# fateshelled/sycl_points

Measured on AMD Instinct MI355X. Metric: gicp_correspondences_per_sec, higher is better.
Workload: dtype f32

## Files before the change

### sycl_points_amd/csrc/registration.hip

```cpp
#include <algorithm>
#include <mutex>

#include "registration_device.h"
#include "sp_cov_normal.h"

namespace sp {
namespace {


struct PointTerm {
    float H[6][6];
    float b[6];
    float sq;
    float residual_norm;
    float genz_weight;
};

__device__ __forceinline__ void se3_jacobian(const Rigid& T, float px, float py, float pz, float J[3][6]) {
#pragma unroll
    for (int i = 0; i < 3; ++i) {
        const float r0 = T.R[i][0], r1 = T.R[i][1], r2 = T.R[i][2];
        J[i][0] = chain3(r0, 0.0f, r1, pz, r2, -py);
        J[i][1] = chain3(r0, -pz, r1, 0.0f, r2, px);
        J[i][2] = chain3(r0, py, r1, -px, r2, 0.0f);
// ... 333 lines not shown
    if ((threadIdx.x & (kWave - 1)) == 0) {
        atomicAdd(&counts[0], inl);
        atomicAdd(&counts[1], pl);
    }
}

__global__ void gn_update_kernel(sp_linearized* lin, float* T, float lambda, float crit_rot, float crit_trans,
                                 float* delta_out8) {
    __shared__ LdltScratch ldlt_ws;
    if (threadIdx.x == 0 && blockIdx.x == 0) gn_update_impl(lin, T, lambda, crit_rot, crit_trans, delta_out8, true, ldlt_ws);
}


template <bool P2D>
__global__ __launch_bounds__(kBlock) void prepare_cov_kernel(const float4* __restrict__ covs, unsigned n,
                                                             const float4* __restrict__ order_pts,
                                                             const unsigned* __restrict__ order_idx,
                                                             float4* __restrict__ out,
                                                             const float* __restrict__ rho2 = nullptr) {
    const unsigned i = blockIdx.x * kBlock + threadIdx.x;
    if (i >= n) return;
    const unsigned src = order_pts ? __float_as_uint(order_pts[i].w) : (order_idx ? order_idx[i] : i);
    const Mat3 C = load_cov(covs + 4 * (size_t)src);
    const Mat3 P = P2D ? inverse(C) : plane_regularize(C);
    out[2 * (size_t)i] = make_float4(P.m[0][0], (P.m[0][1] + P.m[1][0]) * 0.5f, (P.m[0][2] + P.m[2][0]) * 0.5f, P.m[1][1]);
    out[2 * (size_t)i + 1] = make_float4((P.m[1][2] + P.m[2][1]) * 0.5f, P.m[2][2], rho2 ? rho2[src] : 0.0f, 0.0f);
}

__global__ __launch_bounds__(kBlock) void inverse_order_kernel(const float4* __restrict__ gpts, unsigned n,
                                                               unsigned* __restrict__ inv) {
    const unsigned i = blockIdx.x * kBlock + threadIdx.x;
    if (i < n) inv[__float_as_uint(gpts[i].w)] = i;
}
__global__ __launch_bounds__(kBlock) void certificate_kernel(const float4* __restrict__ gpts, unsigned n,
                                                             const int32_t* __restrict__ idx3,
                                                             const float* __restrict__ d23,
                                                             const unsigned* __restrict__ inv,
                                                             float* __restrict__ rho2, float4* __restrict__ nb, float bound2) {
    const unsigned i = blockIdx.x * kBlock + threadIdx.x;
    if (i >= n) return;
    const unsigned o = __float_as_uint(gpts[i].w);
    constexpr float kShrink = 0.25f * (1.0f - 1e-3f);
    rho2[o] = fminf(d23[3 * (size_t)i + 1], bound2) * kShrink;
    const int u1 = idx3[3 * (size_t)i + 1];
    float4 r = make_float4(INFINITY, INFINITY, INFINITY, 0.0f);
    if (u1 >= 0) {
        const float4 p = gpts[inv[u1]];
        r.x = p.x; r.y = p.y; r.z = p.z;
    }
    r.w = fminf(d23[3 * (size_t)i + 2], bound2) * kShrink;
    nb[i] = r;
}

__global__ __launch_bounds__(kBlock) void query_cell_kernel(const float4* __restrict__ pts, unsigned n, GridDesc g,
                                                            Mat4Arg T_val, const float* __restrict__ T_dev,
                                                            unsigned* __restrict__ keys, unsigned* __restrict__ vals) {
    const unsigned i = blockIdx.x * kBlock + threadIdx.x;
    if (i >= n) return;
    const Rigid T = load_rigid_colmajor(T_dev ? T_dev : T_val.m);
    const float4 p = pts[i];
    float qx, qy, qz;
    transform_point(T, p.x, p.y, p.z, qx, qy, qz);
    unsigned key = (unsigned)g.nx * g.ny * g.nz;
    if (isfinite(qx) && isfinite(qy) && isfinite(qz)) {
        const int cx = cell_coord(qx, g.ox, g.inv_h, g.nx), cy = cell_coord(qy, g.oy, g.inv_h, g.ny),
                  cz = cell_coord(qz, g.oz, g.inv_h, g.nz);
        key = ((unsigned)cz * g.ny + cy) * g.nx + cx;
    }
    keys[i] = key;
    vals[i] = i;
}
__global__ __launch_bounds__(kBlock) void prepare_source_kernel(const float4* __restrict__ pts,
                                                                const float4* __restrict__ covs,
                                                                unsigned* __restrict__ order, bool identity, unsigned n,
                                                                float* __restrict__ tiles) {
    const unsigned i = blockIdx.x * kBlock + threadIdx.x;
    if (i >= n) return;
    const unsigned src = identity ? i : order[i];
    if (identity) order[i] = i;
    const float4 p = pts[src];
    float* const w = tiles + ((size_t)(i / kWave) * kSrcTileWords + (i % kWave));
    w[0] = p.x; w[kWave] = p.y; w[2 * kWave] = p.z;
    if (!covs) return;
    const Mat3 P = plane_regularize(load_cov(covs + 4 * (size_t)src));
// ... 208 lines not shown
                xrow[r][e] = ok ? __uint_as_float((unsigned)v) : 0.0f;
            }
            __syncthreads();
            if (s_late) return false;
            if (threadIdx.x < kFanRow) {
                float sum = 0.0f;
                for (int r = 0; r < A.x.world; ++r) sum += xrow[r][threadIdx.x];
                red[1][threadIdx.x] = sum;
            }
        } else {
            const float rv = threadIdx.x < kFanRow ? A.fan_row_in[threadIdx.x] : 0.0f;
            after_loads();
            if (threadIdx.x < kFanRow) red[1][threadIdx.x] = rv;
        }
        __syncthreads();
        if (threadIdx.x < kAcc - 1) red[0][threadIdx.x] = red[1][threadIdx.x];
        else if (threadIdx.x == kAcc - 1)
            red[0][kAcc - 1] = __uint_as_float((unsigned)red[1][kAcc] * 4096u + (unsigned)red[1][kAcc - 1]);
        else if (threadIdx.x == kAcc) red[0][kAcc] = red[1][kAcc + 1];
        __syncthreads();
        return true;
    }
}
__device__ __forceinline__ void align_store_late_state(const AlignArgs& A) {
    if (threadIdx.x < kStateWords) {
        unsigned w = A.has_prev ? reinterpret_cast<const unsigned*>(A.state_in)[threadIdx.x] : 0u;
        if (!A.has_prev && threadIdx.x < 16) w = __float_as_uint(A.T_init[threadIdx.x]);
        if (threadIdx.x == kStateFlagWord) w = 1u;
        if (threadIdx.x == kStateFlagWord + 3) w = 1u;
        reinterpret_cast<unsigned*>(A.state_out)[threadIdx.x] = w;
    }
}

template <bool SHARDED>
__device__ __forceinline__ bool align_prologue(const AlignArgs& A, float* sT, unsigned* sflag) {
    __shared__ float red[kFinalThreads / 32][kPartial];
    __shared__ sp_linearized slin;
    __shared__ float sdelta[8];
    __shared__ LdltScratch ldlt_ws;
    if (A.first) {
        state_store(state_load(false, nullptr, A.T_init), sT, sflag);
        if (!SHARDED && blockIdx.x == 0 && A.searched_log && threadIdx.x >= 64 && threadIdx.x < 64 + kSearchedLog)
            A.searched_log[threadIdx.x - 64] = 0u;
        __syncthreads();
        return true;
    }
    const unsigned sv = state_load(A.has_prev, A.state_in, A.T_init);
    const unsigned nrows = (SHARDED && A.mode == ALIGN_ROWS) ? (unsigned)kAlignMaxBlocks : gridDim.x;
    const bool arrived = align_totals<SHARDED>(A, A.prev_rows, nrows, red, [=] { state_store(sv, sT, sflag); }, sflag);
    if (!arrived) {
        if (blockIdx.x == 0) align_store_late_state(A);
        return false;
    }
    auto zero_row = [&] {
        if (SHARDED && A.mode == ALIGN_FANIN && blockIdx.x == 0 && threadIdx.x >= 64 && threadIdx.x < 64 + kFanRow)
            A.fan_row_out[threadIdx.x - 64] = 0.0f;
    };
    if (sflag[0]) {
        if (blockIdx.x == 0 && threadIdx.x < kStateWords)
            reinterpret_cast<unsigned*>(A.state_out)[threadIdx.x] = reinterpret_cast<const unsigned*>(A.state_in)[threadIdx.x];
        zero_row();
        return false;
    }
    if (threadIdx.x == 0)
        finish_iteration(red[0], sT, A.lambda, A.crit_rot, A.crit_trans, sflag[1], &slin, sdelta, &ldlt_ws, blockIdx.x == 0, A.state_out,
                         A.searched_log,
                         A.k, A.lin_out);
    __syncthreads();
    if (sdelta[6] > 0.5f) {
        zero_row();
        return false;
    }
    return true;
}

template <int LOSS, bool FAST_NN, bool P2D = false, bool SHARDED = false>
__global__ __launch_bounds__(kAlignBlock) void gicp_align_kernel(FusedParams P, AlignArgs A,
                                                                 float* __restrict__ partials) {
    __shared__ float sT[16];
    __shared__ unsigned sflag[2];
    if (!align_prologue<SHARDED>(A, sT, sflag)) return;
    const Rigid T = uniform_pose(sT);
    float acc[kAcc - 1];
    unsigned cnt = 0, searched = 0;
    const unsigned stride = gridDim.x * kAlignBlock;
#pragma unroll
    for (int e = 0; e < kAcc - 1; ++e) acc[e] = 0.0f;
    const unsigned tile = xcd_tile();
    for (unsigned i = tile * kAlignBlock + threadIdx.x; i < P.n; i += stride)
        fused_point<LOSS, FAST_NN, P2D, kSeedSearches, kNegCert>(P, T, i, acc, cnt, searched);
    if constexpr (!SHARDED) {
        block_reduce_store<kAcc - 1, kAlignBlock>(acc, cnt, partials + (size_t)blockIdx.x * kPartial, false, searched);
    } else if (A.mode == ALIGN_ROWS) {
        block_reduce_store<kAcc - 1, kAlignBlock>(acc, cnt, partials + (size_t)blockIdx.x * kPartial, true, searched);
    } else {
        block_reduce_store<kAcc - 1, kAlignBlock, true>(acc, cnt, partials + (size_t)blockIdx.x * kPartial, false, searched);
        align_tail(A, partials);
    }
}

struct PersistArgs {
    AlignWs ws;
    unsigned* tickets;
    const float* T_init;
    float lambda, crit_rot, crit_trans;
    sp_linearized* lin_out;
    float* T_out;
    float* delta_out8;
    uint32_t* iterations_out;
    int max_iterations;
    int k_begin;
    int cache_valid_later;
    unsigned long long budget;
};
template <int LOSS, bool FAST_NN, bool P2D = false>
__global__ __launch_bounds__(kAlignBlock) void gicp_align_persistent_kernel(FusedParams P, PersistArgs A) {
    __shared__ float sT[16];
    __shared__ float red[kFinalThreads / 32][kPartial];
    __shared__ sp_linearized slin;
    __shared__ float sdelta[8];
    __shared__ LdltScratch ldlt_ws;
    __shared__ unsigned s_flag;
    const unsigned stride = gridDim.x * kAlignBlock;
    const unsigned tile = xcd_tile();
    __shared__ unsigned s_prev[2];
    if (A.k_begin >= 2) {
        if (threadIdx.x < 18) {
            const unsigned v = reinterpret_cast<const unsigned*>(&A.ws.state[A.k_begin & 1])[threadIdx.x < 16 ? threadIdx.x : kStateFlagWord + threadIdx.x - 16];
            if (threadIdx.x < 16) sT[threadIdx.x] = __uint_as_float(v);
            else s_prev[threadIdx.x - 16] = v;
        }
    } else {
        if (threadIdx.x < 16) sT[threadIdx.x] = A.T_init[threadIdx.x];
        else if (threadIdx.x < 18) s_prev[threadIdx.x - 16] = 0u;
    }
    if (A.k_begin == 0 && blockIdx.x == 0 && A.ws.searched_log && threadIdx.x >= 64 && threadIdx.x < 64 + kSearchedLog)
        A.ws.searched_log[threadIdx.x - 64] = 0u;
    __syncthreads();
    if (s_prev[0]) {
        if (blockIdx.x == 0) {
            const AlignState* const sp_ = &A.ws.state[A.k_begin & 1];
            if (threadIdx.x < kStateWords)
                reinterpret_cast<unsigned*>(&A.ws.state[(A.k_begin + 1) & 1])[threadIdx.x] = reinterpret_cast<const unsigned*>(sp_)[threadIdx.x];
            if (threadIdx.x < 16) A.T_out[threadIdx.x] = sp_->T[threadIdx.x];
            else if (threadIdx.x < 24 && A.delta_out8) A.delta_out8[threadIdx.x - 16] = sp_->delta[threadIdx.x - 16];
            else if (threadIdx.x == 24 && A.iterations_out) *A.iterations_out = sp_->iterations;
        }
        return;
    }
    unsigned iterations = s_prev[1];
    for (int k = A.k_begin;; ++k) {
        if (k > 0) {
            if (threadIdx.x == 0) s_flag = grid_wait(A.tickets, gridDim.x * (unsigned)(k - A.k_begin), A.budget) ? 0u : 2u;
            __syncthreads();
            if (s_flag == 2) {
                if (blockIdx.x == 0 && threadIdx.x < 16) A.T_out[threadIdx.x] = __int_as_float(0x7fc00000);
                if (blockIdx.x == 0 && threadIdx.x == 16 && A.iterations_out) *A.iterations_out = 0xffffffffu;
                if (blockIdx.x == 0 && threadIdx.x == 17) { A.ws.state[0].pad = 2u; A.ws.state[1].pad = 2u; }
                return;
            }
            reduce_rows_1024<true>(A.ws.part[(k - 1) & 1], gridDim.x, kAcc - 1, red, false, [] {});
            if (threadIdx.x == 0) {
                const bool publish = blockIdx.x == 0;
                AlignState* const so = &A.ws.state[(k - 1) & 1];
                if (publish) {
#pragma unroll
                    for (int i = 0; i < 16; ++i) so->T_lin[i] = sT[i];
                }
                unpack_totals(red[0], kAcc - 1, &slin);
                gn_update_impl(&slin, sT, A.lambda, A.crit_rot, A.crit_trans, sdelta, false, ldlt_ws);
                const bool conv = sdelta[6] > 0.5f;
                const bool last = conv || k == A.max_iterations;
                if (publish) {
                    const unsigned searched = (unsigned)red[0][kAcc];
#pragma unroll
                    for (int i = 0; i < 16; ++i) so->T[i] = sT[i];
#pragma unroll
                    for (int i = 0; i < 8; ++i) so->delta[i] = sdelta[i];
                    so->converged = conv ? 1u : 0u;
                    so->iterations = iterations + 1;
                    so->searched = searched;
                    so->pad = 0;
                    if (A.ws.searched_log && k - 1 < kSearchedLog) A.ws.searched_log[k - 1] = searched;
                    if (A.lin_out) *A.lin_out = slin;
                    if (last) {
                        A.ws.state[k & 1] = *so;
#pragma unroll
                        for (int i = 0; i < 16; ++i) A.T_out[i] = sT[i];
                        if (A.delta_out8)
#pragma unroll
                            for (int i = 0; i < 8; ++i) A.delta_out8[i] = sdelta[i];
                        if (A.iterations_out) *A.iterations_out = iterations + 1;
                    }
                }
                s_flag = last ? 1u : 0u;
            }
            __syncthreads();
            ++iterations;
            if (s_flag) return;
        }
        const Rigid T = uniform_pose(sT);
        float acc[kAcc - 1];
        unsigned cnt = 0, searched = 0;
#pragma unroll
        for (int e = 0; e < kAcc - 1; ++e) acc[e] = 0.0f;
        if (k == 1) P.cache_valid = A.cache_valid_later;
        for (unsigned i = tile * kAlignBlock + threadIdx.x; i < P.n; i += stride)
            fused_point<LOSS, FAST_NN, P2D, kSeedSearches, kNegCert>(P, T, i, acc, cnt, searched);
        block_reduce_store<kAcc - 1, kAlignBlock, true>(acc, cnt, A.ws.part[k & 1] + (size_t)blockIdx.x * kPartial, false, searched);
        grid_arrive(A.tickets);
        if (k == A.max_iterations - 1 && blockIdx.x != 0) return;
    }
}

struct AlignPublish {
    float* T_out;
    float* delta_out8;
    uint32_t* iterations_out;
    unsigned* xchg_epoch;
};
__device__ __forceinline__ void align_publish(const AlignState* state, const AlignPublish& Pb) {
    __threadfence();
    __syncthreads();
    if (!Pb.T_out) return;
    const unsigned* const w = reinterpret_cast<const unsigned*>(state);
    if (threadIdx.x < 16)
        reinterpret_cast<unsigned*>(Pb.T_out)[threadIdx.x] = __hip_atomic_load(w + threadIdx.x, __ATOMIC_RELAXED, __HIP_MEMORY_SCOPE_AGENT);
    else if (threadIdx.x < 24 && Pb.delta_out8)
        reinterpret_cast<unsigned*>(Pb.delta_out8)[threadIdx.x - 16] =
            __hip_atomic_load(w + 32 + (threadIdx.x - 16), __ATOMIC_RELAXED, __HIP_MEMORY_SCOPE_AGENT);
    else if (threadIdx.x == 24 && Pb.iterations_out)
        *Pb.iterations_out = __hip_atomic_load(w + kStateFlagWord + 1, __ATOMIC_RELAXED, __HIP_MEMORY_SCOPE_AGENT);
    else if (threadIdx.x == 32 && Pb.xchg_epoch)
        *Pb.xchg_epoch += 1u;
}
static_assert(offsetof(AlignState, delta) == 4 * 32, "AlignState layout");

__global__ __launch_bounds__(kFinalThreads) void align_solve_kernel(AlignArgs A, const float* __restrict__ rows,
                                                                    unsigned nrows, AlignPublish Pb) {
// ... 167 lines not shown
}
extern "C" int sp_genz_counts(const float* tgt_covs, const int32_t* nn_idx, const float* nn_d2, size_t n, float max_corr,
                              float planarity_threshold, uint32_t* counts_out, void* stream) {
    using namespace sp;
    hipStream_t st = as_stream(stream);
    if (zero_async(counts_out, 8, st) != SP_OK) return SP_ERR_HIP;
    if (n == 0) return SP_OK;
    genz_counts_kernel<<<reduce_grid(n), kBlock, 0, st>>>(reinterpret_cast<const float4*>(tgt_covs), nn_idx, nn_d2,
                                                          (unsigned)n, max_corr * max_corr, planarity_threshold,
                                                          counts_out);
    return launch_status();
}
extern "C" int sp_gn_update(sp_linearized* lin, float* T_dev, float lambda, float crit_rotation, float crit_translation,
                            float* delta_out8, void* stream) {
    sp::gn_update_kernel<<<1, 64, 0, sp::as_stream(stream)>>>(lin, T_dev, lambda, crit_rotation, crit_translation,
                                                              delta_out8);
    return sp::launch_status();
}
extern "C" int sp_gn_update_host(const sp_linearized* lin_host, float* T_host, float lambda, float crit_rotation,
                                 float crit_translation, float* delta_out8_host) {
    sp_linearized tmp = *lin_host;
    sp::LdltScratch w;
    sp::gn_update_impl(&tmp, T_host, lambda, crit_rotation, crit_translation, delta_out8_host, false, w);
    return SP_OK;
}



extern "C" void sp_gicp_target_destroy(sp_gicp_target* t) {
    if (!t) return;
    sp::pooled_free_after(t->covp, t->streams);
    sp::pooled_free_after(t->rho2, t->streams);
    sp::pooled_free_after(t->nb, t->streams);
    delete t;
}
extern "C" int sp_gicp_target_prepare(sp_gicp_target* t, const float* tgt_covs, int reg_type, void* stream) {
    using namespace sp;
    if (!t || !tgt_covs) {
        sp_set_error(reg_type == SP_REG_POINT_TO_DISTRIBUTION
                         ? "[Registration::validate_params] Covariance matrices of target must be pre-computed before "
                           "performing Point-to-Distribution ICP matching."
                         : "[Registration::validate_params] Covariance matrices of source and target must be pre-computed "
                           "before performing GICP matching.");
        return SP_ERR_RUNTIME;
    }
    if (reg_type != SP_REG_GICP && reg_type != SP_REG_POINT_TO_DISTRIBUTION) {
        sp_set_error("[sp_gicp_target_prepare] only RegType::GICP and RegType::POINT_TO_DISTRIBUTION have a prepared form");
        return SP_ERR_INVALID_ARGUMENT;
    }
    ++t->version;
    t->reg_type = reg_type;
    if (t->n == 0) return SP_OK;
    t->note(as_stream(stream));
    const float4* covs = reinterpret_cast<const float4*>(tgt_covs);
    if (reg_type == SP_REG_GICP)
        prepare_cov_kernel<false><<<div_up(t->n, kBlock), kBlock, 0, as_stream(stream)>>>(covs, (unsigned)t->n, t->grid->d_pts,
                                                                                          nullptr, t->covp, t->rho2);
    else
        prepare_cov_kernel<true><<<div_up(t->n, kBlock), kBlock, 0, as_stream(stream)>>>(covs, (unsigned)t->n, t->grid->d_pts,
                                                                                         nullptr, t->covp, t->rho2);
    return launch_status();
}
extern "C" int sp_gicp_target_update(sp_gicp_target* t, const float* tgt_covs, void* stream) {
    return sp_gicp_target_prepare(t, tgt_covs, t ? t->reg_type : SP_REG_GICP, stream);
}
namespace sp {
namespace {
int build_certificates(sp_gicp_target* t, hipStream_t st) {
    const sp_grid* const grid = t->grid;
    const size_t n = t->n;
    if (n == 0 || t->rho2 != nullptr) return SP_OK;
    ScratchBuf b_idx3, b_d23, b_inv;
    hipError_t e = pooled_alloc(&t->rho2, n * sizeof(float), st);
    if (e == hipSuccess) e = pooled_alloc(&t->nb, n * sizeof(float4), st);
    if (e == hipSuccess) e = b_idx3.get(n * 3 * sizeof(int32_t), st);
    if (e == hipSuccess) e = b_d23.get(n * 3 * sizeof(float), st);
    if (e == hipSuccess) e = b_inv.get(n * sizeof(unsigned), st);
    int32_t* const idx3 = b_idx3.as<int32_t>();
    float* const d23 = b_d23.as<float>();
    unsigned* const inv = b_inv.as<unsigned>();
    int rc = e == hipSuccess ? SP_OK : SP_ERR_HIP;
    const float bound2 = 9.0f * grid->h * grid->h;
    if (rc == SP_OK) rc = grid_search_own_points(grid, 3, idx3, d23, st, bound2);
    if (rc == SP_OK) {
        inverse_order_kernel<<<div_up(n, kBlock), kBlock, 0, st>>>(grid->d_pts, (unsigned)n, inv);
        certificate_kernel<<<div_up(n, kBlock), kBlock, 0, st>>>(grid->d_pts, (unsigned)n, idx3, d23, inv, t->rho2, t->nb, bound2);
        rc = launch_status();
    }
    if (hipStreamSynchronize(st) != hipSuccess && rc == SP_OK) rc = SP_ERR_HIP;
    if (rc != SP_OK) {
        if (e != hipSuccess) sp_set_error(hipGetErrorString(e));
        pooled_free(t->rho2); t->rho2 = nullptr;
        pooled_free(t->nb); t->nb = nullptr;
    }
    return rc;
}
int target_create(const sp_grid* grid, const float* tgt_covs, size_t n, bool certificates, void* stream, sp_gicp_target** out) {
    if (!out || !grid) return SP_ERR_INVALID_ARGUMENT;
    *out = nullptr;
    if (grid->n != n) {
        sp_set_error("[sp_gicp_target_create] the grid was built on a cloud of a different size");
        return SP_ERR_INVALID_ARGUMENT;
    }
    sp_gicp_target* t = new sp_gicp_target();
    t->grid = grid;
    t->n = n;
    t->note(as_stream(stream));
    if (n) {
        const hipError_t e = pooled_alloc(&t->covp, n * 2 * sizeof(float4), as_stream(stream));
        if (e != hipSuccess) {
            sp_set_error(hipGetErrorString(e));
            sp_gicp_target_destroy(t);
            return SP_ERR_HIP;
        }
    }
    if (certificates) {
        const int rc2 = build_certificates(t, as_stream(stream));
        if (rc2 != SP_OK) { sp_gicp_target_destroy(t); return rc2; }
    }
    const int rc = sp_gicp_target_update(t, tgt_covs, stream);
    if (rc != SP_OK) { sp_gicp_target_destroy(t); return rc; }
    *out = t;
    return SP_OK;
}
}
}
// ... 517 lines not shown
```

### sycl_points_amd/csrc/registration_device.h

```cpp
#ifndef SP_REGISTRATION_DEVICE_H
#define SP_REGISTRATION_DEVICE_H

#include "grid_device.h"
#include "radix_sort.h"
#include "sp_linearize.h"
#include "sp_xchg.h"

#include <type_traits>

void sp_set_error(const char* msg);

#include "sp_internal.h"

namespace sp {
namespace {

constexpr int kAcc = 29;
constexpr int kPartial = 32;
constexpr int kMaxBlocks = 1024;

template <bool SC1>
__device__ __forceinline__ void store_row_word(float* p, float v) {
    if (SC1) __hip_atomic_store(p, v, __ATOMIC_RELAXED, __HIP_MEMORY_SCOPE_AGENT);
    else *p = v;
}
template <bool SC1>
__device__ __forceinline__ float load_row_word(const float* p) {
    return SC1 ? __hip_atomic_load(p, __ATOMIC_RELAXED, __HIP_MEMORY_SCOPE_AGENT) : *p;
}
template <int NV, int BLOCK = kBlock, bool SC1 = false>
__device__ __forceinline__ void block_reduce_store(float (&acc)[NV], unsigned cnt, float* __restrict__ partial,
                                                   bool count_as_float = false, unsigned extra = 0) {
    __shared__ float red[BLOCK / kWave][kPartial];
    const unsigned lane = threadIdx.x & (kWave - 1), wave = threadIdx.x / kWave;
#pragma unroll
    for (int e = 0; e < NV; ++e) acc[e] = wave_sum_to_lane63(acc[e]);
    cnt = wave_sum_u32_to_lane63(cnt);
// ... 149 lines not shown
    for (int i = 0; i < 6; ++i) {
        H[i * 6 + i] = lin->H[i * 6 + i] + lambda * 1.0f;
        nb[i] = -lin->b[i];
    }
    const bool ok = ldlt6_solve(H, nb, delta, w);
    const float nr = sqrtf(delta[0] * delta[0] + delta[1] * delta[1] + delta[2] * delta[2]);
    const float nt = sqrtf(delta[3] * delta[3] + delta[4] * delta[4] + delta[5] * delta[5]);
    const bool conv = ok && (nr < crit_rot) && (nt < crit_trans);
    const Rigid cur = load_rigid_colmajor(T);
    const Rigid upd = rigid_mul(cur, se3_exp(delta));
    store_rigid_colmajor(upd, T);
    if (delta_out8) {
        for (int i = 0; i < 6; ++i) delta_out8[i] = delta[i];
        delta_out8[6] = conv ? 1.0f : 0.0f;
        delta_out8[7] = ok ? 1.0f : 0.0f;
    }
}

__device__ __forceinline__ Sym3 load_sym(const float4* __restrict__ p) {
    const float4 a = p[0], b = p[1];
    return Sym3{a.x, a.y, a.z, a.w, b.x, b.y};
}

constexpr unsigned kSrcPlanes = 9;
constexpr unsigned kSrcTileWords = kSrcPlanes * kWave;
__host__ __device__ inline size_t src_tile_words(size_t n) { return (n + kWave - 1) / kWave * kSrcTileWords; }

struct FusedParams {
    const float* src;
    const float4* tpts;
    const unsigned* tstart;
    const float4* tcovp;
    const float4* tnb;
    GridDesc g;
    unsigned n;
    float max_d2, scale;
    Mat4Arg T_val;
    const float* T_dev;
    const unsigned* perm;
    float4* ccache;
    int cache_valid;
    int32_t* nn_idx;
    float* nn_d2;
};

__device__ __forceinline__ const float* src_words(const FusedParams& P, unsigned i) {
    return P.src + ((size_t)(i / kWave) * kSrcTileWords + (i % kWave));
}
__device__ __forceinline__ float4 src_point(const float* __restrict__ w) {
    return make_float4(w[0], w[kWave], w[2 * kWave], 1.0f);
}
__device__ __forceinline__ Sym3 src_cov(const float* __restrict__ w) {
    return Sym3{w[3 * kWave], w[4 * kWave], w[5 * kWave], w[6 * kWave], w[7 * kWave], w[8 * kWave]};
}

template <int LOSS, bool P2D = false, bool ERR_ONLY = false, int NACC = kAcc - 1>
__device__ __forceinline__ void fused_math(const FusedParams& P, const Rigid& T, const float4 s, float qx, float qy,
                                           float qz, const Nearest& nn, const Sym3& Cs, const Sym3& Ct,
                                           float (&acc)[NACC], unsigned& cnt) {
    float t[NACC];
    linearize_terms<LOSS, P2D, ERR_ONLY>(T, s.x, s.y, s.z, qx, qy, qz, nn.x, nn.y, nn.z, Cs, Ct, P.scale, t);
#pragma unroll
    for (int e = 0; e < NACC; ++e) acc[e] += t[e];
    ++cnt;
}

// ... 5 lines not shown
    if (nn.idx >= 0) {
        const float4 c0 = P.tcovp[2 * (size_t)nn.pos], c1 = P.tcovp[2 * (size_t)nn.pos + 1];
        r0 = make_float4(nn.x, nn.y, nn.z, c1.z);
        r1 = c0;
        r2 = make_float4(c1.x, c1.y, __int_as_float(nn.idx), __uint_as_float(nn.pos));
        Ct = Sym3{c0.x, c0.y, c0.z, c0.w, c1.x, c1.y};
    }
    row[0] = r0;
    row[1] = r1;
    row[2] = r2;
}

__device__ __forceinline__ bool certified(const FusedParams& P, float d, float rho2, float qx, float qy, float qz,
                                          unsigned pos) {
    if (d < rho2) return true;
    if (!P.tnb || !(rho2 > 0.0f)) return false;
    const float4 nb = P.tnb[pos];
    return d < nb.w && d < dist2(qx, qy, qz, nb.x, nb.y, nb.z);
}

__device__ __forceinline__ float search_bound2(const FusedParams& P) {
    return (P.nn_idx == nullptr && P.max_d2 < FLT_MAX) ? __uint_as_float(__float_as_uint(P.max_d2) + 1u) : FLT_MAX;
}
__device__ __forceinline__ float search_bound2_margin(const FusedParams& P, float& margin2) {
    margin2 = 0.0f;
    if (P.nn_idx != nullptr || !(P.max_d2 < FLT_MAX) || P.ccache == nullptr) return search_bound2(P);
    const float B = sqrtf(P.max_d2), m = 0.25f * B;
    const float wide = (B + m) * (B + m);
    if (!(wide < FLT_MAX)) return search_bound2(P);
    margin2 = (0.98f * m) * (0.98f * m);
    return wide;
}

template <int LOSS, bool FAST_NN, bool P2D = false, bool SEED = true, bool NEG = true>
__device__ __forceinline__ void fused_point(const FusedParams& P, const Rigid& T, unsigned i, float (&acc)[kAcc - 1],
                                            unsigned& cnt, unsigned& searched) {
    const float* const sw = src_words(P, i);
    const float4 s = src_point(sw);
    float4* const row = P.ccache + 3 * (size_t)i;
    float qx, qy, qz;
    transform_point(T, s.x, s.y, s.z, qx, qy, qz);
    Nearest nn;
    Sym3 Ct{0.0f, 0.0f, 0.0f, 0.0f, 0.0f, 0.0f};
    bool hit = false;
    bool seeded = false;
    Nearest seed;
    seed.d2 = FLT_MAX; seed.idx = -1; seed.pos = 0; seed.x = seed.y = seed.z = 0.0f;
    if (P.cache_valid) {
        const float4 r0 = row[0], r1 = row[1], r2 = row[2];
        const float d = dist2(qx, qy, qz, r0.x, r0.y, r0.z);
        const unsigned pos = __float_as_uint(r2.w);
        if (certified(P, d, r0.w, qx, qy, qz, pos)) {
            hit = true;
            nn.idx = __float_as_int(r2.z); nn.pos = pos; nn.x = r0.x; nn.y = r0.y; nn.z = r0.z;
            nn.d2 = nn.idx >= 0 ? d : FLT_MAX;
            Ct = Sym3{r1.x, r1.y, r1.z, r1.w, r2.x, r2.y};
        } else if (SEED && __float_as_int(r2.z) >= 0) {
            seed.d2 = d; seed.idx = __float_as_int(r2.z); seed.pos = pos; seed.x = r0.x; seed.y = r0.y; seed.z = r0.z;
            seeded = true;
        }
    }
    if (!hit) {
        ++searched;
        float margin2 = 0.0f;
        const float bound2 = NEG ? search_bound2_margin(P, margin2) : search_bound2(P);
        seeded = seeded && seed.d2 < bound2;
        if (!seeded) { seed.d2 = bound2; seed.idx = -1; seed.pos = 0; seed.x = seed.y = seed.z = 0.0f; }
        if (FAST_NN) {
            nn = grid_nn1_auto(P.tpts, P.tstart, P.g, qx, qy, qz, bound2, &seed);
        } else {
            nn = grid_nn1(P.tpts, P.tstart, P.g, qx, qy, qz, &seed, 0);
        }
        if (NEG) store_correspondence(row, P, nn, Ct, qx, qy, qz, margin2);
        else store_correspondence(row, P, nn, Ct);
    }
    if (P.nn_idx) {
        const unsigned o = P.perm[i];
        P.nn_idx[o] = nn.idx;
        P.nn_d2[o] = nn.d2;
    }
    if (nn.idx < 0 || nn.d2 > P.max_d2) return;
    unsigned i_again = i;
    asm volatile("" : "+v"(i_again));
    const float* const sw_again = src_words(P, i_again);
    const Sym3 Cs = P2D ? Sym3{0.0f, 0.0f, 0.0f, 0.0f, 0.0f, 0.0f} : src_cov(sw_again);
    fused_math<LOSS, P2D>(P, T, src_point(sw_again), qx, qy, qz, nn, Cs, Ct, acc, cnt);
}

#ifdef SP_OPT_TIMING
__device__ unsigned long long g_sp_dbg[24 * 16];
__device__ unsigned g_sp_step;
__device__ unsigned long long g_sp_wg[24 * 8];
#define SP_PSTAMP(k) if (blockIdx.x == 0 && threadIdx.x == 0 && g_sp_step < 24) g_sp_dbg[g_sp_step * 16 + (k)] = wall_clock64()
#else
#define SP_PSTAMP(k)
#endif
template <int LOSS, bool P2D = false>
__device__ __forceinline__ void fused_point_wave(const FusedParams& P, const Rigid& T, unsigned i, bool valid,
                                                 float (&acc)[kAcc - 1], unsigned& cnt, unsigned& searched) {
    const unsigned ii = valid ? i : 0u;
    SP_PSTAMP(0);
    const float* const sw = src_words(P, ii);
    const float4 s = src_point(sw);
    float qx, qy, qz;
// ... 222 lines not shown
}

constexpr int kTicketShards = 8;
constexpr int kTicketStride = 32;
__device__ __forceinline__ void grid_arrive(unsigned* tickets) {
    if (threadIdx.x < kWave) {
        asm volatile("s_waitcnt vmcnt(0)" ::: "memory");
        if (threadIdx.x == 0)
            __hip_atomic_fetch_add(tickets + (blockIdx.x & (kTicketShards - 1)) * kTicketStride, 1u, __ATOMIC_RELAXED,
                                   __HIP_MEMORY_SCOPE_AGENT);
    }
}
__device__ __forceinline__ bool grid_wait(unsigned* tickets, unsigned want, unsigned long long budget) {
    const unsigned long long t0 = wall_clock64();
    for (;;) {
        unsigned have = 0;
#pragma unroll
        for (int sh = 0; sh < kTicketShards; ++sh)
            have += __hip_atomic_load(tickets + sh * kTicketStride, __ATOMIC_RELAXED, __HIP_MEMORY_SCOPE_AGENT);
        if (have >= want) return true;
        if (wall_clock64() - t0 > budget) return false;
        __builtin_amdgcn_s_sleep(2);
    }
}

}
}

struct sp_gicp_target {
    const sp_grid* grid = nullptr;
    float4* covp = nullptr;
    float* rho2 = nullptr;
    float4* nb = nullptr;
    unsigned long long version = 0;
    int reg_type = SP_REG_GICP;
    size_t n = 0;
    mutable sp::StreamSet streams;
    void note(hipStream_t st) const { streams.note(st); if (grid) sp::grid_use(grid, st); }
};
namespace sp {
constexpr size_t kOptRowsBytes = 2 * (size_t)256 * 32 * sizeof(unsigned long long);
}
struct sp_gicp_source {
    size_t n_max = 0, n = 0;
    float* tiles = nullptr;
    unsigned* perm = nullptr;
    float4* ccache = nullptr;
    float4* qcert = nullptr;
    float4* qcert2 = nullptr;
    size_t qcert_points = 0;
    mutable bool qcert_valid = false;
    float4* ccache2 = nullptr;
    unsigned long long* opt_rows = nullptr;
    mutable unsigned opt_epoch = 0;
    mutable bool cache_valid = false;
    const sp_gicp_target* cache_target = nullptr;
    unsigned long long cache_version = 0;
    bool sorted = false;
    int opt_stage_mask = 3;
    int opt_reuse = 2;
    int opt_fast_nn = -1;
    int opt_persistent = 1;
    int opt_persistent_from = 4;
    int opt_fuse_trials = 1;
    int opt_wave_query = 1;
    unsigned *keys_in = nullptr, *keys_out = nullptr, *vals_in = nullptr;
    void* sort_tmp = nullptr;
    size_t sort_tmp_bytes = 0;
};

namespace sp {
namespace {
FusedParams make_fused_params(const sp_gicp_target* target, const sp_gicp_source* source, const sp_factor_params* params,
                              const float* transT, int transT_on_device, int32_t* nn_idx_out, float* nn_d2_out) {
    const size_t n = source->n;
    FusedParams P;
    P.src = source->tiles;
    P.tpts = target->grid->d_pts;
    P.tstart = target->grid->d_start;
    P.tcovp = target->covp;
    P.tnb = source->opt_reuse > 1 ? target->nb : nullptr;
    P.g = grid_desc(target->grid);
    P.n = (unsigned)n;
    P.max_d2 = params->max_correspondence_distance * params->max_correspondence_distance;
    P.scale = params->robust_scale;
    for (int i = 0; i < 16; ++i) P.T_val.m[i] = (i % 5 == 0) ? 1.0f : 0.0f;
    if (transT && !transT_on_device)
        for (int i = 0; i < 16; ++i) P.T_val.m[i] = transT[i];
    P.T_dev = transT_on_device ? transT : nullptr;
    P.perm = source->perm;
    P.ccache = source->ccache;
    P.cache_valid = (source->opt_reuse && source->cache_valid && source->cache_target == target &&
                     source->cache_version == target->version) ? 1 : 0;
    P.nn_idx = (nn_idx_out && nn_d2_out) ? nn_idx_out : nullptr;
    P.nn_d2 = nn_d2_out;
    return P;
}

int check_prepared_reg(const sp_gicp_target* target, const sp_factor_params* params) {
    if (params->reg_type != SP_REG_GICP && params->reg_type != SP_REG_POINT_TO_DISTRIBUTION) {
        sp_set_error("[sp_gicp_*] only RegType::GICP and RegType::POINT_TO_DISTRIBUTION have a prepared/fused form");
        return SP_ERR_INVALID_ARGUMENT;
    }
    if (params->reg_type != target->reg_type) {
        sp_set_error("[sp_gicp_*] the prepared target holds the rows of another RegType: call sp_gicp_target_prepare");
        return SP_ERR_INVALID_ARGUMENT;
    }
    if (params->rotation_constraint_enable) {
        sp_set_error("[sp_gicp_*] the rotation constraint needs the raw covariances: use sp_gicp_linearize");
        return SP_ERR_INVALID_ARGUMENT;
    }
    return SP_OK;
}

// ... 79 lines not shown
```

### sycl_points_amd/csrc/registration_opt.hip

```cpp
#include <algorithm>

#include "sp_optimizer.h"

namespace sp {
namespace {

struct OptArgs {
    float* part[2];
    unsigned* tickets;
    unsigned long long* trows[2];
    unsigned tag_base;
    float4* rows[2];
    float4* qcert[2];
    int qcert_trusted;
    int fuse;
    const float* T_init;
    float* T_out;
    sp_opt_params opt;
    float scales[SP_OPT_MAX_LEVELS];
    int n_levels;
    int reuse;
    sp_align_result* result;
    unsigned long long budget;
};
// ... 162 lines not shown
#endif
    for (unsigned step = 0;; ++step) {
        const int phase = S.ctl.phase;
#ifdef SP_OPT_TIMING
        if (publish && threadIdx.x == 0) g_sp_step = step;
        __syncthreads();
#endif
        SP_STAMP(0);
        SP_WG_BEGIN();
        float* const row = A.part[step & 1] + (size_t)blockIdx.x * kPartial;
        [[maybe_unused]] float mine = 0.0f;
        if constexpr (WAVEQ) P.ccache = A.rows[S.ctl.cur];
        if (phase == PHASE_LIN) {
            P.scale = A.scales[S.ctl.level];
            P.cache_valid = S.ctl.cache_valid;
            const Rigid T = uniform_pose(S.sT);
            float acc[kAcc - 1];
            unsigned cnt = 0, searched = 0;
#pragma unroll
            for (int e = 0; e < kAcc - 1; ++e) acc[e] = 0.0f;
            if constexpr (WAVEQ) {
                const unsigned nw = BLOCK / kWave;
                const unsigned wave = (unsigned)__builtin_amdgcn_readfirstlane((int)(threadIdx.x / kWave));
                const bool qc_trust = A.qcert_trusted || S.ctl.n_lin > 0;
                for (unsigned i = blockIdx.x * nw + wave; i < P.n; i += gridDim.x * nw)
                    fused_query_wave<LOSS, P2D>(P, T, i, acc, cnt, searched, nullptr, qc_trust ? A.qcert[S.ctl.cur] : nullptr, A.qcert[S.ctl.cur]);
                SP_STAMP(4);
                mine = waveq_row_slot<kAcc - 1, BLOCK>(acc, cnt, searched, red);
            } else if constexpr (FAST_NN && BLOCK <= 256) {
                for (unsigned b = tile * BLOCK; b < P.n; b += stride)
                    fused_point_wave<LOSS, P2D>(P, T, b + threadIdx.x, b + threadIdx.x < P.n, acc, cnt, searched);
            } else {
                for (unsigned i = tile * BLOCK + threadIdx.x; i < P.n; i += stride)
                    fused_point<LOSS, FAST_NN, P2D, kSeedSearches, kNegCert>(P, T, i, acc, cnt, searched);
            }
            if constexpr (!WAVEQ) {
                SP_STAMP(4);
                if (single) block_reduce_lds<kAcc - 1, BLOCK>(acc, cnt, searched, red[0]);
                else block_reduce_store<kAcc - 1, BLOCK, true>(acc, cnt, row, false, searched);
            }
        } else if (WAVEQ && phase == PHASE_FUSED) {
            if constexpr (WAVEQ) {
                const Rigid T = uniform_pose(S.sTt);
                const Rigid TL = uniform_pose(S.sTlin);
                float acc[kAcc - 1], acc_t[1] = {0.0f};
                unsigned cnt = 0, searched = 0, cnt_t = 0;
#pragma unroll
                for (int e = 0; e < kAcc - 1; ++e) acc[e] = 0.0f;
                float4* const rows_out = A.rows[S.ctl.cur ^ 1];
                const float scale_trial = A.scales[S.ctl.level], scale_lin = A.scales[S.ctl.spec_level];
                const int reuse = S.reuse;
                const unsigned nw = BLOCK / kWave;
                const unsigned wave = (unsigned)__builtin_amdgcn_readfirstlane((int)(threadIdx.x / kWave));
                for (unsigned i = blockIdx.x * nw + wave; i < P.n; i += gridDim.x * nw) {
                    P.scale = scale_trial;
                    error_prepared_point<LOSS, P2D>(P, T, TL, i, acc_t, cnt_t);
                    P.scale = scale_lin;
                    P.cache_valid = reuse;
                    fused_query_wave<LOSS, P2D>(P, T, i, acc, cnt, searched, rows_out, A.qcert[S.ctl.cur], A.qcert[S.ctl.cur ^ 1]);
                }
                SP_STAMP(4);
                mine = waveq_row_slot<kAcc - 1, BLOCK>(acc, cnt, searched, red, acc_t[0], cnt_t);
            }
        } else {
            const Rigid T = uniform_pose(S.sTt);
            const Rigid TL = uniform_pose(S.sTlin);
            P.scale = A.scales[S.ctl.level];
// ... 207 lines not shown
```

Before: 32.09 billion.

## Add neighbor-list certificate to re-resolve cached correspondences without grid search

Target preparation now runs a self-kNN with more neighbors and records each target point's three nearest neighbors plus a certified radius. During alignment, a cached correspondence that fails the simple certificate can switch to a closer listed neighbor, or be kept, without a full grid NN search. The list path is enabled only when a per-iteration bound on pose change is small relative to the cell size. The default reuse level is raised so the path is on by default. In exchange it adds target-prep work, memory, and extra loads and branches per point.

```diff
diff --git a/sycl_points_amd/csrc/registration.hip b/sycl_points_amd/csrc/registration.hip
--- a/sycl_points_amd/csrc/registration.hip
+++ b/sycl_points_amd/csrc/registration.hip
@@ -389,24 +389,38 @@
     const unsigned i = blockIdx.x * kBlock + threadIdx.x;
     if (i < n) inv[__float_as_uint(gpts[i].w)] = i;
 }
+constexpr int kSelfK = kListK + 2;
 __global__ __launch_bounds__(kBlock) void certificate_kernel(const float4* __restrict__ gpts, unsigned n,
-                                                             const int32_t* __restrict__ idx3,
-                                                             const float* __restrict__ d23,
+                                                             const int32_t* __restrict__ idxs,
+                                                             const float* __restrict__ d2s,
                                                              const unsigned* __restrict__ inv,
-                                                             float* __restrict__ rho2, float4* __restrict__ nb, float bound2) {
+                                                             float* __restrict__ rho2, float4* __restrict__ nb,
+                                                             float4* __restrict__ rec, float bound2) {
     const unsigned i = blockIdx.x * kBlock + threadIdx.x;
     if (i >= n) return;
     const unsigned o = __float_as_uint(gpts[i].w);
     constexpr float kShrink = 0.25f * (1.0f - 1e-3f);
-    rho2[o] = fminf(d23[3 * (size_t)i + 1], bound2) * kShrink;
-    const int u1 = idx3[3 * (size_t)i + 1];
-    float4 r = make_float4(INFINITY, INFINITY, INFINITY, 0.0f);
-    if (u1 >= 0) {
-        const float4 p = gpts[inv[u1]];
-        r.x = p.x; r.y = p.y; r.z = p.z;
-    }
-    r.w = fminf(d23[3 * (size_t)i + 2], bound2) * kShrink;
-    nb[i] = r;
+    const int32_t* const ri = idxs + kSelfK * (size_t)i;
+    const float* const rd = d2s + kSelfK * (size_t)i;
+    rho2[o] = fminf(rd[1], bound2) * kShrink;
+    int self = kSelfK;
+#pragma unroll
+    for (int s = kSelfK - 1; s >= 0; --s)
+        if (ri[s] == (int)o) self = s;
+    float4 u[kListK + 1];
+    unsigned upos[kListK + 1];
+    float ud2[kListK + 1];
+    bool found[kListK + 1];
+#pragma unroll
+    for (int j = 0; j <= kListK; ++j) {
+        const int s = j < self ? j : j + 1;
+        const int id = ri[s];
+        found[j] = id >= 0;
+        upos[j] = found[j] ? inv[id] : 0u;
+        u[j] = gpts[upos[j]];
+        ud2[j] = rd[s];
+    }
+    list_record(nb + i, rec + kListRestVec * (size_t)i, u, upos, ud2, found, bound2);
 }
 
 __global__ __launch_bounds__(kBlock) void query_cell_kernel(const float4* __restrict__ pts, unsigned n, GridDesc g,
@@ -681,8 +695,19 @@
     }
 }
 
+__device__ __forceinline__ float list_step_bound(const float* delta6, const GridDesc& g) {
+    const float cx = fmaxf(fabsf(g.ox), fabsf(g.ox + g.nx * g.h)), cy = fmaxf(fabsf(g.oy), fabsf(g.oy + g.ny * g.h)),
+                cz = fmaxf(fabsf(g.oz), fabsf(g.oz + g.nz * g.h));
+    return sqrtf(chain3(delta6[3], delta6[3], delta6[4], delta6[4], delta6[5], delta6[5])) +
+           sqrtf(chain3(delta6[0], delta6[0], delta6[1], delta6[1], delta6[2], delta6[2])) * sqrtf(chain3(cx, cx, cy, cy, cz, cz));
+}
+__device__ __forceinline__ int list_certificate_pays(float step, const GridDesc& g) {
+    return __builtin_amdgcn_readfirstlane(4.0f * step < g.h ? 1 : 0);
+}
+
 template <bool SHARDED>
-__device__ __forceinline__ bool align_prologue(const AlignArgs& A, float* sT, unsigned* sflag) {
+__device__ __forceinline__ bool align_prologue(const AlignArgs& A, float* sT, unsigned* sflag, float* s_step = nullptr,
+                                               const GridDesc* g = nullptr) {
     __shared__ float red[kFinalThreads / 32][kPartial];
     __shared__ sp_linearized slin;
     __shared__ float sdelta[8];
@@ -691,6 +716,7 @@
         state_store(state_load(false, nullptr, A.T_init), sT, sflag);
         if (!SHARDED && blockIdx.x == 0 && A.searched_log && threadIdx.x >= 64 && threadIdx.x < 64 + kSearchedLog)
             A.searched_log[threadIdx.x - 64] = 0u;
+        if (s_step && threadIdx.x == 0) *s_step = FLT_MAX;
         __syncthreads();
         return true;
     }
@@ -711,10 +737,12 @@
         zero_row();
         return false;
     }
-    if (threadIdx.x == 0)
+    if (threadIdx.x == 0) {
         finish_iteration(red[0], sT, A.lambda, A.crit_rot, A.crit_trans, sflag[1], &slin, sdelta, &ldlt_ws, blockIdx.x == 0, A.state_out,
                          A.searched_log,
                          A.k, A.lin_out);
+        if (s_step) *s_step = list_step_bound(sdelta, *g);
+    }
     __syncthreads();
     if (sdelta[6] > 0.5f) {
         zero_row();
@@ -728,7 +756,11 @@
                                                                  float* __restrict__ partials) {
     __shared__ float sT[16];
     __shared__ unsigned sflag[2];
-    if (!align_prologue<SHARDED>(A, sT, sflag)) return;
+    __shared__ float s_step;
+    if (!align_prologue<SHARDED>(A, sT, sflag, SHARDED ? nullptr : &s_step, &P.g)) return;
+    if constexpr (!SHARDED) {
+        if (P.tlist) P.tlist = list_certificate_pays(s_step, P.g);
+    }
     const Rigid T = uniform_pose(sT);
     float acc[kAcc - 1];
     unsigned cnt = 0, searched = 0;
@@ -737,7 +769,7 @@
     for (int e = 0; e < kAcc - 1; ++e) acc[e] = 0.0f;
     const unsigned tile = xcd_tile();
     for (unsigned i = tile * kAlignBlock + threadIdx.x; i < P.n; i += stride)
-        fused_point<LOSS, FAST_NN, P2D, kSeedSearches, kNegCert>(P, T, i, acc, cnt, searched);
+        fused_point<LOSS, FAST_NN, P2D, kSeedSearches, kNegCert, !SHARDED>(P, T, i, acc, cnt, searched);
     if constexpr (!SHARDED) {
         block_reduce_store<kAcc - 1, kAlignBlock>(acc, cnt, partials + (size_t)blockIdx.x * kPartial, false, searched);
     } else if (A.mode == ALIGN_ROWS) {
@@ -798,6 +830,7 @@
         return;
     }
     unsigned iterations = s_prev[1];
+    const int tlist = P.tlist;
     for (int k = A.k_begin;; ++k) {
         if (k > 0) {
             if (threadIdx.x == 0) s_flag = grid_wait(A.tickets, gridDim.x * (unsigned)(k - A.k_begin), A.budget) ? 0u : 2u;
@@ -854,6 +887,7 @@
 #pragma unroll
         for (int e = 0; e < kAcc - 1; ++e) acc[e] = 0.0f;
         if (k == 1) P.cache_valid = A.cache_valid_later;
+        if (k > 0 && tlist) P.tlist = list_certificate_pays(list_step_bound(sdelta, P.g), P.g);
         for (unsigned i = tile * kAlignBlock + threadIdx.x; i < P.n; i += stride)
             fused_point<LOSS, FAST_NN, P2D, kSeedSearches, kNegCert>(P, T, i, acc, cnt, searched);
         block_reduce_store<kAcc - 1, kAlignBlock, true>(acc, cnt, A.ws.part[k & 1] + (size_t)blockIdx.x * kPartial, false, searched);
@@ -1087,6 +1121,7 @@
     sp::pooled_free_after(t->covp, t->streams);
     sp::pooled_free_after(t->rho2, t->streams);
     sp::pooled_free_after(t->nb, t->streams);
+    sp::pooled_free_after(t->rec, t->streams);
     delete t;
 }
 extern "C" int sp_gicp_target_prepare(sp_gicp_target* t, const float* tgt_covs, int reg_type, void* stream) {
@@ -1128,18 +1163,19 @@
     ScratchBuf b_idx3, b_d23, b_inv;
     hipError_t e = pooled_alloc(&t->rho2, n * sizeof(float), st);
     if (e == hipSuccess) e = pooled_alloc(&t->nb, n * sizeof(float4), st);
-    if (e == hipSuccess) e = b_idx3.get(n * 3 * sizeof(int32_t), st);
-    if (e == hipSuccess) e = b_d23.get(n * 3 * sizeof(float), st);
+    if (e == hipSuccess) e = pooled_alloc(&t->rec, n * kListRestVec * sizeof(float4), st);
+    if (e == hipSuccess) e = b_idx3.get(n * kSelfK * sizeof(int32_t), st);
+    if (e == hipSuccess) e = b_d23.get(n * kSelfK * sizeof(float), st);
     if (e == hipSuccess) e = b_inv.get(n * sizeof(unsigned), st);
     int32_t* const idx3 = b_idx3.as<int32_t>();
     float* const d23 = b_d23.as<float>();
     unsigned* const inv = b_inv.as<unsigned>();
     int rc = e == hipSuccess ? SP_OK : SP_ERR_HIP;
     const float bound2 = 9.0f * grid->h * grid->h;
-    if (rc == SP_OK) rc = grid_search_own_points(grid, 3, idx3, d23, st, bound2);
+    if (rc == SP_OK) rc = grid_search_own_points(grid, kSelfK, idx3, d23, st, bound2);
     if (rc == SP_OK) {
         inverse_order_kernel<<<div_up(n, kBlock), kBlock, 0, st>>>(grid->d_pts, (unsigned)n, inv);
-        certificate_kernel<<<div_up(n, kBlock), kBlock, 0, st>>>(grid->d_pts, (unsigned)n, idx3, d23, inv, t->rho2, t->nb, bound2);
+        certificate_kernel<<<div_up(n, kBlock), kBlock, 0, st>>>(grid->d_pts, (unsigned)n, idx3, d23, inv, t->rho2, t->nb, t->rec, bound2);
         rc = launch_status();
     }
     if (hipStreamSynchronize(st) != hipSuccess && rc == SP_OK) rc = SP_ERR_HIP;
@@ -1147,6 +1183,7 @@
         if (e != hipSuccess) sp_set_error(hipGetErrorString(e));
         pooled_free(t->rho2); t->rho2 = nullptr;
         pooled_free(t->nb); t->nb = nullptr;
+        pooled_free(t->rec); t->rec = nullptr;
     }
     return rc;
 }
diff --git a/sycl_points_amd/csrc/registration_device.h b/sycl_points_amd/csrc/registration_device.h
--- a/sycl_points_amd/csrc/registration_device.h
+++ b/sycl_points_amd/csrc/registration_device.h
@@ -3,6 +3,7 @@
 
 #include "grid_device.h"
 #include "radix_sort.h"
+#include "sp_certificate.h"
 #include "sp_linearize.h"
 #include "sp_xchg.h"
 
@@ -218,6 +219,8 @@
     const unsigned* tstart;
     const float4* tcovp;
     const float4* tnb;
+    const float4* trec;
+    int tlist;
     GridDesc g;
     unsigned n;
     float max_d2, scale;
@@ -289,7 +292,7 @@
     return wide;
 }
 
-template <int LOSS, bool FAST_NN, bool P2D = false, bool SEED = true, bool NEG = true>
+template <int LOSS, bool FAST_NN, bool P2D = false, bool SEED = true, bool NEG = true, bool LIST = true>
 __device__ __forceinline__ void fused_point(const FusedParams& P, const Rigid& T, unsigned i, float (&acc)[kAcc - 1],
                                             unsigned& cnt, unsigned& searched) {
     const float* const sw = src_words(P, i);
@@ -300,6 +303,7 @@
     Nearest nn;
     Sym3 Ct{0.0f, 0.0f, 0.0f, 0.0f, 0.0f, 0.0f};
     bool hit = false;
+    bool moved = false;
     bool seeded = false;
     Nearest seed;
     seed.d2 = FLT_MAX; seed.idx = -1; seed.pos = 0; seed.x = seed.y = seed.z = 0.0f;
@@ -307,26 +311,44 @@
         const float4 r0 = row[0], r1 = row[1], r2 = row[2];
         const float d = dist2(qx, qy, qz, r0.x, r0.y, r0.z);
         const unsigned pos = __float_as_uint(r2.w);
-        if (certified(P, d, r0.w, qx, qy, qz, pos)) {
+        const int tidx = __float_as_int(r2.z);
+        int what = d < r0.w ? LIST_STANDS : LIST_NONE;
+        if (what == LIST_NONE && P.tnb && r0.w > 0.0f) {
+            if (LIST && P.tlist && tidx >= 0) {
+                const ListVerdict v = list_certificate(P.tnb + pos, P.trec + kListRestVec * (size_t)pos, true, qx, qy, qz, r0.x, r0.y, r0.z,
+                                                       pos, d, search_bound2(P));
+                what = v.what;
+                if (what == LIST_MOVED) {
+                    nn.pos = v.pos; nn.x = v.x; nn.y = v.y; nn.z = v.z; nn.d2 = v.d2;
+                    nn.idx = __float_as_int(P.tpts[v.pos].w);
+                    moved = true;
+                }
+            } else if (certified(P, d, r0.w, qx, qy, qz, pos)) {
+                what = LIST_STANDS;
+            }
+        }
+        if (what == LIST_STANDS) {
             hit = true;
-            nn.idx = __float_as_int(r2.z); nn.pos = pos; nn.x = r0.x; nn.y = r0.y; nn.z = r0.z;
+            nn.idx = tidx; nn.pos = pos; nn.x = r0.x; nn.y = r0.y; nn.z = r0.z;
             nn.d2 = nn.idx >= 0 ? d : FLT_MAX;
             Ct = Sym3{r1.x, r1.y, r1.z, r1.w, r2.x, r2.y};
-        } else if (SEED && __float_as_int(r2.z) >= 0) {
-            seed.d2 = d; seed.idx = __float_as_int(r2.z); seed.pos = pos; seed.x = r0.x; seed.y = r0.y; seed.z = r0.z;
+        } else if (SEED && !moved && tidx >= 0) {
+            seed.d2 = d; seed.idx = tidx; seed.pos = pos; seed.x = r0.x; seed.y = r0.y; seed.z = r0.z;
             seeded = true;
         }
     }
     if (!hit) {
-        ++searched;
         float margin2 = 0.0f;
-        const float bound2 = NEG ? search_bound2_margin(P, margin2) : search_bound2(P);
-        seeded = seeded && seed.d2 < bound2;
-        if (!seeded) { seed.d2 = bound2; seed.idx = -1; seed.pos = 0; seed.x = seed.y = seed.z = 0.0f; }
-        if (FAST_NN) {
-            nn = grid_nn1_auto(P.tpts, P.tstart, P.g, qx, qy, qz, bound2, &seed);
-        } else {
-            nn = grid_nn1(P.tpts, P.tstart, P.g, qx, qy, qz, &seed, 0);
+        if (!moved) {
+            ++searched;
+            const float bound2 = NEG ? search_bound2_margin(P, margin2) : search_bound2(P);
+            seeded = seeded && seed.d2 < bound2;
+            if (!seeded) { seed.d2 = bound2; seed.idx = -1; seed.pos = 0; seed.x = seed.y = seed.z = 0.0f; }
+            if (FAST_NN) {
+                nn = grid_nn1_auto(P.tpts, P.tstart, P.g, qx, qy, qz, bound2, &seed);
+            } else {
+                nn = grid_nn1(P.tpts, P.tstart, P.g, qx, qy, qz, &seed, 0);
+            }
         }
         if (NEG) store_correspondence(row, P, nn, Ct, qx, qy, qz, margin2);
         else store_correspondence(row, P, nn, Ct);
@@ -615,6 +637,7 @@
     float4* covp = nullptr;
     float* rho2 = nullptr;
     float4* nb = nullptr;
+    float4* rec = nullptr;
     unsigned long long version = 0;
     int reg_type = SP_REG_GICP;
     size_t n = 0;
@@ -641,7 +664,7 @@
     unsigned long long cache_version = 0;
     bool sorted = false;
     int opt_stage_mask = 3;
-    int opt_reuse = 2;
+    int opt_reuse = 3;
     int opt_fast_nn = -1;
     int opt_persistent = 1;
     int opt_persistent_from = 4;
@@ -663,6 +686,8 @@
     P.tstart = target->grid->d_start;
     P.tcovp = target->covp;
     P.tnb = source->opt_reuse > 1 ? target->nb : nullptr;
+    P.trec = target->rec;
+    P.tlist = (source->opt_reuse > 2 && target->rec != nullptr) ? 1 : 0;
     P.g = grid_desc(target->grid);
     P.n = (unsigned)n;
     P.max_d2 = params->max_correspondence_distance * params->max_correspondence_distance;
diff --git a/sycl_points_amd/csrc/registration_opt.hip b/sycl_points_amd/csrc/registration_opt.hip
--- a/sycl_points_amd/csrc/registration_opt.hip
+++ b/sycl_points_amd/csrc/registration_opt.hip
@@ -218,7 +218,7 @@
                     fused_point_wave<LOSS, P2D>(P, T, b + threadIdx.x, b + threadIdx.x < P.n, acc, cnt, searched);
             } else {
                 for (unsigned i = tile * BLOCK + threadIdx.x; i < P.n; i += stride)
-                    fused_point<LOSS, FAST_NN, P2D, kSeedSearches, kNegCert>(P, T, i, acc, cnt, searched);
+                    fused_point<LOSS, FAST_NN, P2D, kSeedSearches, kNegCert, false>(P, T, i, acc, cnt, searched);
             }
             if constexpr (!WAVEQ) {
                 SP_STAMP(4);
diff --git a/sycl_points_amd/csrc/sp_certificate.h b/sycl_points_amd/csrc/sp_certificate.h
--- /dev/null
+++ b/sycl_points_amd/csrc/sp_certificate.h
@@ -0,0 +1,73 @@
+#pragma once
+#include "sp_math.h"
+
+namespace sp {
+
+constexpr int kListK = 3;
+constexpr int kListRestVec = 3;
+enum { LIST_NONE = 0, LIST_STANDS = 1, LIST_MOVED = 2 };
+
+struct ListVerdict {
+    int what;
+    unsigned pos;
+    float x, y, z;
+    float d2;
+};
+
+SP_HD void list_record(float4* first, float4* rest, const float4* u, const unsigned* upos, const float* ud2, const bool* found,
+                       float bound2) {
+    constexpr float kInf = __builtin_huge_valf();
+    constexpr float kShrink2 = 0.25f * (1.0f - 1e-3f), kShrink = 1.0f - 1e-3f;
+    float4 c[kListK];
+#pragma unroll
+    for (int j = 0; j < kListK; ++j)
+        c[j] = found[j] ? make_float4(u[j].x, u[j].y, u[j].z, 0.0f) : make_float4(kInf, kInf, kInf, 0.0f);
+    const float half2 = fminf(found[1] ? ud2[1] : FLT_MAX, bound2) * kShrink2;
+    const float radius = sqrtf(fminf(found[kListK] ? ud2[kListK] : FLT_MAX, bound2)) * kShrink;
+    auto bits = [](unsigned v) {
+        float f;
+        __builtin_memcpy(&f, &v, 4);
+        return f;
+    };
+    first[0] = make_float4(c[0].x, c[0].y, c[0].z, half2);
+    rest[0] = make_float4(c[1].x, c[1].y, c[1].z, radius);
+    rest[1] = make_float4(c[2].x, c[2].y, c[2].z, bits(found[0] ? upos[0] : 0u));
+    rest[2] = make_float4(bits(found[1] ? upos[1] : 0u), bits(found[2] ? upos[2] : 0u), 0.0f, 0.0f);
+}
+
+SP_HD ListVerdict list_certificate(const float4* first, const float4* rest, bool list, float qx, float qy, float qz, float tx,
+                                   float ty, float tz, unsigned tpos, float d, float bound2) {
+    ListVerdict v;
+    v.what = LIST_NONE; v.pos = tpos; v.x = tx; v.y = ty; v.z = tz; v.d2 = d;
+    const float4 a = first[0];
+    const float d1 = dist2(qx, qy, qz, a.x, a.y, a.z);
+    if (d < a.w && d < d1) {
+        v.what = LIST_STANDS;
+        return v;
+    }
+    if (!list) return v;
+    const float4 b = rest[0], c = rest[1], e = rest[2];
+    const float dt = sqrtf(d);
+    if (!(dt < b.w)) return v;
+    const float d2 = dist2(qx, qy, qz, b.x, b.y, b.z), d3 = dist2(qx, qy, qz, c.x, c.y, c.z);
+    auto word = [](float f) {
+        unsigned w;
+        __builtin_memcpy(&w, &f, 4);
+        return w;
+    };
+    float best = d;
+    if (d1 < best) { best = d1; v.what = LIST_MOVED; v.pos = word(c.w); v.x = a.x; v.y = a.y; v.z = a.z; }
+    if (d2 < best) { best = d2; v.what = LIST_MOVED; v.pos = word(e.x); v.x = b.x; v.y = b.y; v.z = b.z; }
+    if (d3 < best) { best = d3; v.what = LIST_MOVED; v.pos = word(e.y); v.x = c.x; v.y = c.y; v.z = c.z; }
+    if (v.what == LIST_NONE) v.what = LIST_STANDS;
+    const int at_best = (d == best ? 1 : 0) + (d1 == best ? 1 : 0) + (d2 == best ? 1 : 0) + (d3 == best ? 1 : 0);
+    const bool proven = at_best == 1 && sqrtf(best) + dt < b.w && best < bound2;
+    if (!proven) {
+        v.what = LIST_NONE; v.pos = tpos; v.x = tx; v.y = ty; v.z = tz; v.d2 = d;
+        return v;
+    }
+    v.d2 = best;
+    return v;
+}
+
+}
```

Result: no change. 32.37 billion (median of 6 runs) (+0.9%).
